# mika314/melonix

Measured on AMD Instinct MI355X. Metric: STFT+pitch+resynth frames/sec (48 kHz, 4096 FFT, 256 hop); % HBM roofline, higher is better.
Workload: dtype f32

## Files before the change

melonix_amd/csrc/stft_core.h:

```cpp
#pragma once
#include <stdint.h>
#include <type_traits>

#if defined(__HIPCC__)
#include <hip/hip_runtime.h>
#define MX_HD __host__ __device__ __forceinline__
namespace mx {
using cpx = float2;
}
#else
#define MX_HD inline __attribute__((always_inline))
namespace mx {
struct alignas(8) cpx {
  float x, y;
};
}
#endif

namespace mx {

#include "stft_consts.inc"

MX_HD cpx mk(float x, float y) {
  cpx r;
// ... 44 lines not shown
  constexpr int k = ((K % 64) + 64) % 64;
  if constexpr (k == 0) {
    pk_bfly_1(E, O, out0, out1);
  } else if constexpr (k == 16) {
    pk_bfly_mi(E, O, out0, out1);
  } else if constexpr (k == 32) {
    pk_bfly_1(E, O, out1, out0);
  } else if constexpr (k == 48) {
    pk_bfly_mi(E, O, out1, out0);
  } else {
    pk_bfly_cs(E, O, mk(kCos64[k], kSin64[k]), out0, out1);
  }
}

template <int R, int Q>
struct Combine {
  static MX_HD void run(const cpx *E, const cpx *O, cpx *out) {
    bfly_w64<Q * 64 / R>(E[Q], O[Q], out[Q], out[Q + R / 2]);
    if constexpr (Q + 1 < R / 2) Combine<R, Q + 1>::run(E, O, out);
  }
};

template <int R>
struct Dft {
  static MX_HD void run(const cpx *in, cpx *out) {
    cpx e[R / 2], o[R / 2], E[R / 2], O[R / 2];
#pragma unroll
    for (int q = 0; q < R / 2; ++q) {
      e[q] = in[2 * q];
      o[q] = in[2 * q + 1];
    }
    Dft<R / 2>::run(e, E);
    Dft<R / 2>::run(o, O);
    Combine<R, 0>::run(E, O, out);
  }
};
template <>
struct Dft<2> {
  static MX_HD void run(const cpx *in, cpx *out) {
    pk_bfly_1(in[0], in[1], out[0], out[1]);
  }
};
template <>
struct Dft<1> {
  static MX_HD void run(const cpx *in, cpx *out) { out[0] = in[0]; }
};

template <int R, int S, int O0, bool CONJ>
struct DftTw {
  static MX_HD void run(const cpx *v, const cpx *w, cpx *out) {
    if constexpr (R == 2) {
      constexpr int i0 = O0, i1 = O0 + S;
      if constexpr (i0 == 0) pk_leaf0_tw<CONJ>(v[0], v[i1], w[i1], out[0], out[1]);
      else pk_leaf_tw<CONJ>(v[i0], w[i0], v[i1], w[i1], out[0], out[1]);
    } else {
      cpx E[R / 2], O[R / 2];
      DftTw<R / 2, 2 * S, O0, CONJ>::run(v, w, E);
      DftTw<R / 2, 2 * S, O0 + S, CONJ>::run(v, w, O);
      Combine<R, 0>::run(E, O, out);
    }
  }
};

template <int N_, int E_>
struct Plan {
  static constexpr int N = N_;
  static constexpr int M = N / 2;
  static constexpr int E = E_;
  static constexpr int T = M / E;
  static constexpr int R3 = E / 2;
  static constexpr int R1 = (N == 4096) ? 16 : 32;
  static constexpr int R2 = M / (R1 * R3);
  static constexpr int NS3 = R1 * R2;
  static constexpr int NB1 = E / R1;
  static constexpr int NB2 = E / R2;
  static constexpr int TW2 = (R2 - 1) * R1;
  static constexpr int TW3 = (R3 - 1) * NS3;
  static constexpr int L1 = ilog2(R1);
  static_assert(N == 4096 || N == 16384 || N == 32768, "supported FFT sizes");
  static_assert((N == 4096) ? E == 16 : E == 32, "supported points per thread");
  static_assert(R1 * R2 * R3 == M && R2 <= E && R1 <= E && T % 64 == 0, "radix plan must cover M");
};

template <class P>
MX_HD constexpr bool t1_padded() { return P::R1 == 32; }
template <class P>
MX_HD constexpr int t1_size() { return t1_padded<P>() ? P::M + P::M / 32 : P::M; }
template <class P>
MX_HD int t1_index(int i) {
  if constexpr (t1_padded<P>()) return i + (i >> 5);
  else return i ^ ((i >> P::L1) & 15);
}

struct alignas(4) f2u {
  float x, y;
};
template <bool ALIGNED8>
MX_HD cpx ld_pair(const float *base, int i) {
  const char *a = reinterpret_cast<const char *>(base) + (size_t)(4u * (unsigned)i);
  if constexpr (ALIGNED8) {
    return *reinterpret_cast<const cpx *>(a);
  } else {
    const f2u u = *reinterpret_cast<const f2u *>(a);
    return mk(u.x, u.y);
  }
}

MX_HD float ld_one(const float *base, int i) {
  return *reinterpret_cast<const float *>(reinterpret_cast<const char *>(base) + (size_t)(4u * (unsigned)i));
}

template <class P, int WSTEP, bool ALIGNED8>
MX_HD void load_frame(int t, cpx (&Y)[P::E], const float *x, const float *w) {
#pragma unroll
  for (int e = 0; e < P::E; ++e) {
    const int p = 2 * (t + P::T * e);
    cpx xs, ws;
    if constexpr (ALIGNED8 && WSTEP == 1) {
      xs = ld_pair<true>(x, p);
      ws = ld_pair<true>(w, p);
    } else {
      xs = ld_pair<false>(x, p);
      if constexpr (WSTEP == 1) {
        ws = ld_pair<false>(w, p);
      } else {
        const f2u wu = *reinterpret_cast<const f2u *>(w - p - 1);
        ws = mk(wu.y, wu.x);
      }
    }
    Y[e] = pk_mul(xs, ws);
  }
}

template <int T>
MX_HD constexpr float win_grow(int e) {
  return T == 64 ? kWinGrow64[e] : T == 128 ? kWinGrow128[e] : T == 256 ? kWinGrow256[e] : kWinGrow512[e];
}
template <class P, bool CLAMP = true>
MX_HD cpx geo_weight(cpx a0, int e) {
  constexpr float sc = 0.5f / (float)P::N;
  const float g = e == 0 ? 1.0f : win_grow<P::T>(e);
  const cpx w = e == 0 ? a0 : mk(a0.x * g, a0.y * g);
  if constexpr (!CLAMP) {
    return w;
  } else {
    const unsigned sb = __builtin_bit_cast(unsigned, sc), xb = __builtin_bit_cast(unsigned, w.x), yb = __builtin_bit_cast(unsigned, w.y);
    return mk(__builtin_bit_cast(float, xb < sb ? xb : sb), __builtin_bit_cast(float, yb < sb ? yb : sb));
  }
}
template <class P>
MX_HD int geo_clamped_slots(int hop) { return (hop + 2 * P::T - 1) / (2 * P::T); }
constexpr int kGeoTail = 2;
template <class P, bool ALIGNED8>
MX_HD void load_frame_geo(int t, cpx (&Y)[P::E], const float *x, const float *wb, int hop) {
  static_assert(P::T == 64 || P::T == 128 || P::T == 256 || P::T == 512, "growth table per T");
  static_assert(P::E <= 32, "growth table length");
  const cpx a0 = ld_pair<true>(wb, 2 * t);
  if (geo_clamped_slots<P>(hop) <= kGeoTail) {
#pragma unroll
    for (int e = 0; e < P::E; ++e) {
      const cpx xs = ld_pair<ALIGNED8>(x, 2 * (t + P::T * e));
      Y[e] = pk_mul(xs, e < P::E - kGeoTail ? geo_weight<P, false>(a0, e) : geo_weight<P, true>(a0, e));
    }
  } else {
#pragma unroll
    for (int e = 0; e < P::E; ++e) Y[e] = pk_mul(ld_pair<ALIGNED8>(x, 2 * (t + P::T * e)), geo_weight<P, true>(a0, e));
  }
}

template <class P>
MX_HD void apply_window_geo(int t, cpx (&Y)[P::E], const cpx (&xr)[P::E], const float *wb, int hop) {
  const cpx a0 = ld_pair<true>(wb, 2 * t);
  if (geo_clamped_slots<P>(hop) <= kGeoTail) {
#pragma unroll
    for (int e = 0; e < P::E; ++e)
      Y[e] = pk_mul(xr[e], e < P::E - kGeoTail ? geo_weight<P, false>(a0, e) : geo_weight<P, true>(a0, e));
  } else {
#pragma unroll
    for (int e = 0; e < P::E; ++e) Y[e] = pk_mul(xr[e], geo_weight<P, true>(a0, e));
  }
}

template <class P, bool ALIGNED8>
MX_HD void load_raw(int t, cpx (&xr)[P::E], const float *x) {
#pragma unroll
  for (int e = 0; e < P::E; ++e) {
    xr[e] = ld_pair<ALIGNED8>(x, 2 * (t + P::T * e));
  }
}
template <class P, int WSTEP, bool ALIGNED8>
MX_HD void apply_window(int t, cpx (&Y)[P::E], const cpx (&xr)[P::E], const float *w) {
#pragma unroll
  for (int e = 0; e < P::E; ++e) {
    const int p = 2 * (t + P::T * e);
    cpx ws;
    if constexpr (WSTEP == 1) {
      ws = ld_pair<ALIGNED8>(w, p);
    } else {
      const f2u wu = *reinterpret_cast<const f2u *>(w - p - 1);
      ws = mk(wu.y, wu.x);
    }
    Y[e] = pk_mul(xr[e], ws);
  }
}

template <class P>
MX_HD void pass1(const cpx (&Y)[P::E], cpx (&v)[P::E]) {
#pragma unroll
  for (int b = 0; b < P::NB1; ++b) {
    cpx in[P::R1], out[P::R1];
#pragma unroll
    for (int r = 0; r < P::R1; ++r) in[r] = Y[b + P::NB1 * r];
    Dft<P::R1>::run(in, out);
#pragma unroll
    for (int r = 0; r < P::R1; ++r) v[b * P::R1 + r] = out[r];
  }
}

template <class P, int HOP>
struct Slide {
  static constexpr int H = HOP / 2;
  static constexpr bool ok = (HOP > 0) && (HOP % 2 == 0) && (H % P::T == 0) && (2 * (H / P::T) <= P::E);
  static constexpr int D = ok ? H / P::T : 1;
};

template <class P, int HOP>
MX_HD void slide_edge(int t, const float *wtab, float inv_sc, cpx (&edge)[Slide<P, HOP>::D]) {
  using S = Slide<P, HOP>;
#pragma unroll
  for (int i = 0; i < S::D; ++i) {
    const int p = 2 * (t + P::T * (P::E - 2 * S::D + i));
    edge[i] = mk(wtab[p] * inv_sc, wtab[p + 1] * inv_sc);
  }
}

template <class P, int HOP>
MX_HD void slide_fetch(int t, const float *xe, cpx (&nx)[Slide<P, HOP>::D]) {
  using S = Slide<P, HOP>;
#pragma unroll
  for (int i = 0; i < S::D; ++i) nx[i] = *reinterpret_cast<const cpx *>(xe - HOP + 2 * (t + P::T * i));
}

template <class P, int HOP>
MX_HD void slide_step(cpx (&Y)[P::E], const cpx (&nx)[Slide<P, HOP>::D], const cpx (&edge)[Slide<P, HOP>::D],
                      float g, float sc) {
  using S = Slide<P, HOP>;
  const cpx gg = mk(g, g), ss = mk(sc, sc);
#pragma unroll
  for (int e = 0; e < P::E - 2 * S::D; ++e) Y[e] = pk_mul_xs(Y[e + S::D], gg);
#pragma unroll
  for (int i = 0; i < S::D; ++i) Y[P::E - 2 * S::D + i] = pk_mul(Y[P::E - S::D + i], edge[i]);
#pragma unroll
  for (int i = 0; i < S::D; ++i) Y[P::E - S::D + i] = pk_mul_xs(nx[i], ss);
}


template <class P>
struct Circ {
  static constexpr int W = 2 * P::T;
  static constexpr int CS = (P::T == 128) ? 4 : (P::T == 256) ? 3 : 2;
  static MX_HD bool ok(int hop) { return hop >= 1 && hop <= (CS - 1) * P::T && hop <= 2 * W; }
  static constexpr int slot(int k) { return (P::E - (CS - 1) + k) & (P::E - 1); }
};
template <class P>
struct CircGeo {
  int o;
  int s;
  int cr;
  int len;
};
template <class P>
MX_HD CircGeo<P> circ_geo(long long frame_end, int hop) {
  constexpr int W = Circ<P>::W;
  const long long start = frame_end - P::N;
  CircGeo<P> g;
  g.o = (int)(start & (long long)(W - 1));
  g.s = ((int)((start - hop) & (long long)(W - 1)) + hop) / W;
  g.len = 2 * hop;
  g.cr = (g.o - g.len) & (P::N - 1);
  return g;
}
template <class P>
MX_HD void circ_load_first(int t, cpx (&Y)[P::E], const float *xa, const float *w, int o) {
#pragma unroll
  for (int e = 0; e < P::E; ++e) {
    const int c2 = 2 * (t + P::T * e);
    const int q0 = (c2 - o) & (P::N - 1), q1 = (c2 + 1 - o) & (P::N - 1);
    Y[e] = mk(xa[q0] * w[q0], xa[q1] * w[q1]);
  }
}
template <class P>
MX_HD void circ_fetch(int t, const float *xs, const float *wt, const CircGeo<P> &g, float (&px)[2 * Circ<P>::CS],
                      float (&pw)[2 * Circ<P>::CS]) {
#pragma unroll
  for (int k = 0; k < Circ<P>::CS; ++k) {
    const int c2 = 2 * (t + P::T * Circ<P>::slot(k));
    int d0 = (c2 - g.cr) & (P::N - 1), d1 = (c2 + 1 - g.cr) & (P::N - 1);
    d0 = d0 < g.len ? d0 : g.len - 1;
    d1 = d1 < g.len ? d1 : g.len - 1;
    px[2 * k] = ld_one(xs, d0);
    px[2 * k + 1] = ld_one(xs, d1);
    pw[2 * k] = ld_one(wt, d0);
    pw[2 * k + 1] = ld_one(wt, d1);
  }
}
template <class P, int S>
MX_HD void circ_age(cpx (&Y)[P::E], cpx gg) {
  cpx head[S > 0 ? S : 1];
#pragma unroll
  for (int i = 0; i < S; ++i) head[i] = Y[i];
#pragma unroll
  for (int e = 0; e < P::E - S; ++e) Y[e] = pk_mul_xs(Y[e + S], gg);
#pragma unroll
  for (int i = 0; i < S; ++i) Y[P::E - S + i] = pk_mul_xs(head[i], gg);
}
template <class P>
MX_HD void circ_step(int t, cpx (&Y)[P::E], float decay, const CircGeo<P> &g, const float (&px)[2 * Circ<P>::CS],
                     const float (&pw)[2 * Circ<P>::CS]) {
  const cpx gg = mk(decay, decay);
  constexpr int SMAX = (Circ<P>::W - 1 + (Circ<P>::CS - 1) * P::T) / Circ<P>::W;
  static_assert(SMAX <= 2, "rotations by 0, 1 or 2 slots");
  if (g.s == 0) circ_age<P, 0>(Y, gg);
  else if (SMAX == 1 || g.s == 1) circ_age<P, 1>(Y, gg);
  else circ_age<P, 2>(Y, gg);
#pragma unroll
  for (int k = 0; k < Circ<P>::CS; ++k) {
    const int e = Circ<P>::slot(k);
    const int c2 = 2 * (t + P::T * e);
    const int d0 = (c2 - g.cr) & (P::N - 1), d1 = (c2 + 1 - g.cr) & (P::N - 1);
    const float n0 = px[2 * k] * pw[2 * k], n1 = px[2 * k + 1] * pw[2 * k + 1];
    Y[e] = mk(d0 < g.len ? n0 : Y[e].x, d1 < g.len ? n1 : Y[e].y);
  }
}


#if defined(__HIP_DEVICE_COMPILE__)
#define MX_LDS_ASM 1
typedef float mx_f2v __attribute__((ext_vector_type(2)));
template <int OFF>
__device__ __forceinline__ mx_f2v lds_rd64(uint32_t addr) {
  static_assert(OFF >= 0 && OFF < 163840, "LDS is 160 KiB");
  mx_f2v r;
  if constexpr (OFF < 65536) {
    asm volatile("ds_read_b64 %0, %1 offset:%2" : "=v"(r) : "v"(addr), "n"(OFF) : "memory");
  } else {
    const uint32_t hi = addr + (uint32_t)(OFF & ~65535);
    asm volatile("ds_read_b64 %0, %1 offset:%2" : "=v"(r) : "v"(hi), "n"(OFF & 65535) : "memory");
  }
  return r;
}
__device__ __forceinline__ uint32_t lds_addr(const void *p) {
  return (uint32_t)(uintptr_t)(const __attribute__((address_space(3))) void *)p;
}
template <int N>
__device__ __forceinline__ void lds_wait(mx_f2v (&q)[N]) {
  static_assert(N % 8 == 0, "tied in groups of 8");
  asm volatile("s_waitcnt lgkmcnt(0)" ::: "memory");
#pragma unroll
  for (int i = 0; i < N; i += 8)
    asm volatile("" : "+v"(q[i]), "+v"(q[i + 1]), "+v"(q[i + 2]), "+v"(q[i + 3]), "+v"(q[i + 4]),
                 "+v"(q[i + 5]), "+v"(q[i + 6]), "+v"(q[i + 7]));
}
#endif
template <int I, int N, class F>
MX_HD void static_for(F &&f) {
  if constexpr (I < N) {
    f(std::integral_constant<int, I>{});
    static_for<I + 1, N>(f);
  }
}

template <class P>
MX_HD void store_t1(int t, const cpx (&v)[P::E], cpx *lds) {
  if constexpr (t1_padded<P>()) {
    static_assert(P::R1 <= 32 && (P::T * P::R1) % 32 == 0, "T1 padding is one point per 32");
    cpx *const p = lds + (t * P::R1 + ((t * P::R1) >> 5));
#pragma unroll
    for (int b = 0; b < P::NB1; ++b) {
#pragma unroll
      for (int r = 0; r < P::R1; ++r) p[b * (P::T * P::R1 + P::T * P::R1 / 32) + r] = v[b * P::R1 + r];
    }
  } else {
    const unsigned B8 = (unsigned)((t * P::R1) ^ (t & 15)) << 3;
    char *const base = reinterpret_cast<char *>(lds);
#pragma unroll
    for (int r = 0; r < P::R1; ++r) {
      cpx *p = reinterpret_cast<cpx *>(base + (B8 ^ ((unsigned)r << 3)));
#pragma unroll
      for (int b = 0; b < P::NB1; ++b) p[b * P::T * P::R1] = v[b * P::R1 + r];
    }
  }
}

template <class P>
struct T1Read {
  static constexpr int S = P::M / P::R2;
  static constexpr int SP = t1_padded<P>() ? S + S / 32 : S;
  static constexpr int TP = t1_padded<P>() ? P::T + P::T / 32 : P::T;
  static constexpr int step = t1_padded<P>() ? 0 : ((S >> P::L1) & 15);
  static_assert(S % 32 == 0 && P::T % 32 == 0 && (step == 0 || step == 8), "T1 read is base(+alt base) + offset");
  static_assert(t1_padded<P>() || P::NB2 == 1, "the XOR layout's bases are written for one pass-2 butterfly per thread");
};

template <class P>
MX_HD void load_t1(int t, cpx (&v)[P::E], const cpx *lds) {
  using R = T1Read<P>;
  const int s1 = t1_index<P>(t);
#ifdef MX_LDS_ASM
  mx_f2v q[P::E];
  const uint32_t ae = lds_addr(lds + s1), ao = lds_addr(lds + (s1 ^ R::step));
  static_for<0, P::NB2>([&](auto bb) {
    constexpr int b = decltype(bb)::value;
    static_for<0, P::R2>([&](auto rr) {
      constexpr int r = decltype(rr)::value;
      q[b * P::R2 + r] = lds_rd64<(b * R::TP + r * R::SP) * 8>((r & 1) ? ao : ae);
    });
  });
  lds_wait(q);
#pragma unroll
  for (int i = 0; i < P::E; ++i) v[i] = mk(q[i].x, q[i].y);
#else
  const cpx *pe = lds + s1, *po = lds + (s1 ^ R::step);
#pragma unroll
  for (int b = 0; b < P::NB2; ++b) {
#pragma unroll
    for (int r = 0; r < P::R2; ++r) v[b * P::R2 + r] = ((r & 1) ? po : pe)[b * R::TP + r * R::SP];
  }
#endif
}

template <class P>
MX_HD void load_t1_tw2(int t, cpx (&v)[P::E], const cpx *lds, const cpx *ltw2, cpx (&w)[P::R2 - 1]) {
  static_assert(P::NB2 == 1 && P::E == P::R2 && P::E % 8 == 0, "one pass-2 butterfly per thread");
  using R = T1Read<P>;
  const int s1 = t1_index<P>(t);
#ifdef MX_LDS_ASM
  const uint32_t ae = lds_addr(lds + s1), ao = lds_addr(lds + (s1 ^ R::step));
  const uint32_t aw = lds_addr(ltw2 + (t & (P::R1 - 1)));
  mx_f2v q[2 * P::E];
  static_for<0, P::R2>([&](auto rr) {
    constexpr int r = decltype(rr)::value;
    q[r] = lds_rd64<r * R::SP * 8>((r & 1) ? ao : ae);
  });
  static_for<1, P::R2>([&](auto rr) {
    constexpr int r = decltype(rr)::value;
    q[P::E + r] = lds_rd64<(r - 1) * P::R1 * 8>(aw);
  });
  q[P::E] = mx_f2v{0.0f, 0.0f};
  lds_wait(q);
#pragma unroll
  for (int i = 0; i < P::E; ++i) v[i] = mk(q[i].x, q[i].y);
#pragma unroll
  for (int r = 1; r < P::R2; ++r) w[r - 1] = mk(q[P::E + r].x, q[P::E + r].y);
#else
  const cpx *pe = lds + s1, *po = lds + (s1 ^ R::step), *pw = ltw2 + (t & (P::R1 - 1));
#pragma unroll
  for (int r = 0; r < P::R2; ++r) v[r] = ((r & 1) ? po : pe)[r * R::SP];
#pragma unroll
  for (int r = 1; r < P::R2; ++r) w[r - 1] = pw[(r - 1) * P::R1];
#endif
}

template <class P>
MX_HD void pass2(int t, cpx (&v)[P::E], const cpx *tw2) {
#pragma unroll
  for (int b = 0; b < P::NB2; ++b) {
    const int j = t + P::T * b;
    const int k = j & (P::R1 - 1);
    cpx in[P::R2], w[P::R2], out[P::R2];
    w[0] = mk(1.0f, 0.0f);
#pragma unroll
    for (int r = 0; r < P::R2; ++r) in[r] = v[b * P::R2 + r];
#pragma unroll
    for (int r = 1; r < P::R2; ++r) {
      w[r] = tw2[(r - 1) * P::R1 + k];
    }
    DftTw<P::R2, 1, 0, false>::run(in, w, out);
#pragma unroll
    for (int r = 0; r < P::R2; ++r) v[b * P::R2 + r] = out[r];
  }
}

template <class P>
MX_HD void pass2_reg(cpx (&v)[P::E], const cpx (&w)[P::R2 - 1]) {
  static_assert(P::NB2 == 1, "one pass-2 butterfly per thread");
  cpx in[P::R2], ww[P::R2], out[P::R2];
  ww[0] = mk(1.0f, 0.0f);
#pragma unroll
  for (int r = 0; r < P::R2; ++r) in[r] = v[r];
#pragma unroll
  for (int r = 1; r < P::R2; ++r) ww[r] = w[r - 1];
  DftTw<P::R2, 1, 0, false>::run(in, ww, out);
#pragma unroll
  for (int r = 0; r < P::R2; ++r) v[r] = out[r];
}

template <class P>
MX_HD void store_t2(int t, const cpx (&v)[P::E], cpx *lds) {
#pragma unroll
  for (int b = 0; b < P::NB2; ++b) {
    const int j = t + P::T * b;
    const int k = j & (P::R1 - 1);
    const int base = (j - k) * P::R2 + k;
    cpx *p = lds + base;
#pragma unroll
    for (int r = 0; r < P::R2; ++r) p[r * P::R1] = v[b * P::R2 + r];
  }
}

template <class P>
MX_HD int k0p(int t) { return t; }
template <class P>
MX_HD int k0q(int t) { return t ? P::NS3 - t : P::NS3 / 2; }

template <class P>
MX_HD void load_t2(int t, cpx (&v)[P::E], const cpx *lds) {
  const int p = k0p<P>(t), q = k0q<P>(t);
#ifdef MX_LDS_ASM
  {
    const uint32_t pa = lds_addr(lds + p), qa = lds_addr(lds + q);
    mx_f2v w[P::E];
    static_for<0, P::R3>([&](auto rr) {
      constexpr int r = decltype(rr)::value;
      w[r] = lds_rd64<P::NS3 * r * 8>(pa);
      w[P::R3 + r] = lds_rd64<P::NS3 * r * 8>(qa);
    });
    lds_wait(w);
#pragma unroll
    for (int i = 0; i < P::E; ++i) v[i] = mk(w[i].x, w[i].y);
  }
#else
  const cpx *pp = lds + p, *qq = lds + q;
#pragma unroll
  for (int r = 0; r < P::R3; ++r) {
    v[r] = pp[P::NS3 * r];
    v[P::R3 + r] = qq[P::NS3 * r];
// ... 242 lines not shown
```

melonix_amd/csrc/stft_kernel_impl.h:

```cpp
#pragma once
#include <hip/hip_runtime.h>

#include "colormap_core.h"
#include "kernels.h"
#include "stft_core.h"
#include "stft_tables.h"

#define MX_BARRIER() __syncthreads()

namespace mx {

template <bool MAXOP>
__device__ __forceinline__ unsigned wave_reduce_u32(unsigned k) {
  constexpr unsigned ident = MAXOP ? 0u : 0xffffffffu;
#define MX_DPP_STEP(CTRL, ROWS)                                                                      \
  {                                                                                                  \
    const unsigned o = (unsigned)__builtin_amdgcn_update_dpp((int)ident, (int)k, CTRL, ROWS, 0xf, false); \
    k = MAXOP ? (o > k ? o : k) : (o < k ? o : k);                                                   \
  }
  MX_DPP_STEP(0xB1, 0xf)
  MX_DPP_STEP(0x4E, 0xf)
  MX_DPP_STEP(0x141, 0xf)
  MX_DPP_STEP(0x140, 0xf)
  MX_DPP_STEP(0x142, 0xa)
  MX_DPP_STEP(0x143, 0xc)
#undef MX_DPP_STEP
  return (unsigned)__builtin_amdgcn_readlane((int)k, 63);
}
__device__ __forceinline__ unsigned long long wave_max_u64(unsigned long long k) {
  const unsigned hi = (unsigned)(k >> 32), lo = (unsigned)k;
  const unsigned mhi = wave_reduce_u32<true>(hi);
  const unsigned long long tie = __ballot(hi == mhi);
  unsigned mlo;
  if (__builtin_popcountll(tie) == 1) mlo = (unsigned)__builtin_amdgcn_readlane((int)lo, __builtin_ctzll(tie));
  else mlo = wave_reduce_u32<true>(hi == mhi ? lo : 0u);
  return ((unsigned long long)mhi << 32) | mlo;
}

template <int IMM, bool NT = true>
__device__ __forceinline__ void st_row_nt(const float *base, unsigned off, float x) {
  static_assert(IMM >= -4096 && IMM <= 4095, "global_store immediate offset");
#if defined(__HIP_DEVICE_COMPILE__)
  if constexpr (NT) asm volatile("global_store_dword %0, %1, %2 offset:%3 nt" : : "v"(off), "v"(x), "s"(base), "n"(IMM) : "memory");
  else asm volatile("global_store_dword %0, %1, %2 offset:%3" : : "v"(off), "v"(x), "s"(base), "n"(IMM) : "memory");
#endif
}

template <class P, int MODE, int HOP, int WPE, bool DEFER = false, bool PREFETCH = false, bool CMAP = false, bool DIRECT = false,
          bool CIRC = false, bool ROWPICK = false>
__global__ __launch_bounds__(P::T) __attribute__((amdgpu_waves_per_eu(WPE, WPE)))
void stft_kernel(const StftArgs a0) {
  const StftArgs &a = a0;
  using C = P;
  constexpr int N = P::N;
  constexpr int NW = C::T / 64;
  constexpr int kRed = (NW > 1) ? ((NW + 1) / 2) * 2 : 0;
  constexpr bool kTw3Bases = (P::R3 == 16);
  constexpr int kTw2 = ((C::TW2 + 1) / 2) * 2;
  static_assert(P::R3 == 16 || P::R3 == 8, "twiddle placement per plan");
  static_assert(!DIRECT || (NW > 1 && !DEFER && !CMAP), "direct row stores: multi-wave, non-deferred plans");
  static_assert(!ROWPICK || (DEFER && NW > 1 && !CMAP && !DIRECT && C::M / 4 / C::T >= 1 && C::T >= 128),
                "row-side pitch pick: the deferred two-wave plan, rows without texels");
  static_assert(!CIRC || (MODE != kRanges && HOP == 0 && !PREFETCH && !CMAP), "circular window: bulk modes");
  constexpr int IMG = t1_size<C>();
  __shared__ __attribute__((aligned(16))) float2 lds[IMG + kRed + (DEFER ? C::M / 2 : 0) + kTw2];
  float *const lout = reinterpret_cast<float *>(DEFER ? lds + IMG : lds);
  float2 *const ltw2 = lds + IMG + kRed + (DEFER ? C::M / 2 : 0);

  const int t_ = threadIdx.x;
  constexpr bool kSlide = (MODE == kBulkAligned) && (HOP > 0) && Slide<P, (HOP > 0 ? HOP : 2)>::ok;
  constexpr int SD = Slide<P, (HOP > 0 ? HOP : 2)>::D;
  const bool wave0 = __builtin_amdgcn_readfirstlane(t_) < 64;
  cpx u[kTw3Bases ? 1 : P::R3];
  cpx ulo;
  cpx w3r[kTw3Bases ? 1 : P::R3 - 1], w3base[6];
  if constexpr (kTw3Bases) {
    cpx uhi_unused;
    post_bases<P>(t_, a.ubase, ulo, uhi_unused);
    fetch_tw3_bases<P>(t_, a.tw3, w3base);
  } else {
    post_twiddles<P>(t_, a.ubase, *reinterpret_cast<cpx(*)[P::R3]>(&u));
    fetch_tw3<P>(t_, a.tw3, *reinterpret_cast<cpx(*)[P::R3 - 1]>(&w3r));
  }
  constexpr int kTw3Hoist = (!kTw3Bases && ROWPICK) ? ((kSlide && SD > 1) ? 3 : P::R3 - 1) : 0;
  cpx w3p[kTw3Hoist > 0 ? kTw3Hoist : 1];
  if constexpr (!kTw3Bases) pass3_wp0<P, kTw3Hoist>(t_, *reinterpret_cast<cpx(*)[P::R3 - 1]>(&w3r), w3p);
  uint32_t bmask_ = 0;
  uint32_t umask = 0;
  if constexpr (!ROWPICK) {
    bmask_ = band_mask<P>(t_, a.kmin, a.kmax);
#pragma unroll
    for (int o = 0; o < P::E; ++o) umask |= (__ballot((bmask_ >> o) & 1u) != 0ull) ? (1u << o) : 0u;
    umask = __builtin_amdgcn_readfirstlane(umask);
  }
  unsigned long long rin[4] = {0ull, 0ull, 0ull, 0ull};
  if constexpr (ROWPICK) {
    const unsigned rm = row_band_mask(4 * t_, a.kmin, a.kmax);
#pragma unroll
    for (int j = 0; j < 4; ++j) rin[j] = __ballot((rm >> j) & 1u);
  }
  constexpr float kSc = 0.5f / (float)N;
  for (int i = t_; i < C::TW2; i += C::T) ltw2[i] = a.tw2[i];
  MX_BARRIER();

  unsigned lb = blockIdx.x;
  {
    const unsigned nb = gridDim.x, xcd = lb & 7u, q = nb >> 3, r = nb & 7u;
    lb = (xcd < r ? xcd * (q + 1) : r * (q + 1) + (xcd - r) * q) + (lb >> 3);
  }
  const int64_t f0 = (int64_t)lb * a.frames_per_block;
  const int64_t f1 = (f0 + a.frames_per_block < a.count) ? f0 + a.frames_per_block : a.count;

  cpx Y[P::E];
  cpx edge[SD], nx[SD];
  if constexpr (kSlide) {
    const int64_t e0 = (a.first_frame + f0 + 1) * (int64_t)HOP;
    if (f0 < f1) load_frame<P, 1, true>(t_, Y, a.audio + MX_AUDIO_PAD + (e0 - N), a.wtab);
    slide_edge<P, HOP>(t_, a.wtab, 2.0f * (float)N, edge);
  }

  unsigned long long *const red = reinterpret_cast<unsigned long long *>(lds + IMG + (DEFER ? C::M / 2 : 0));
  auto flush_pitch = [&](int64_t fr, int tt) {
    if (!ROWPICK && a.pitch && tt == 0) {
      unsigned long long b = red[0];
#pragma unroll
      for (int i = 1; i < NW; ++i) b = red[i] > b ? red[i] : b;
      mx_pitch p;
      p.bin = 0x7fffffff - (int)(unsigned)(b & 0xffffffffull);
      p.mag = __uint_as_float((unsigned)(b >> 32));
      a.pitch[fr] = p;
    }
  };
  const bool want_rows = a.mags != nullptr || (CMAP && a.rgb != nullptr);
  constexpr bool kRowSaddr = (C::M / 4 / C::T == 4) && (C::T * 16 == 2048);
  auto flush_row = [&](int64_t fr, int tt) {
    if (want_rows) {
      using f32x4 = float __attribute__((ext_vector_type(4)));
      const f32x4 *l4 = reinterpret_cast<const f32x4 *>(lout) + tt;
      f32x4 *row4 = reinterpret_cast<f32x4 *>(a.mags + (size_t)fr * (size_t)(N / 2)) + tt;
      f32x4 q[C::M / 4 / C::T];
#pragma unroll
      for (int i = 0; i < C::M / 4 / C::T; ++i) q[i] = l4[C::T * i];
      if (!CMAP || a.mags) {
        if constexpr (kRowSaddr) {
          uintptr_t mid = reinterpret_cast<uintptr_t>(a.mags + (size_t)fr * (size_t)(N / 2)) + 4096;
#if defined(__HIP_DEVICE_COMPILE__)
          asm volatile("" : "+s"(mid));
          using gchar = __attribute__((address_space(1))) char;
          using gf32x4 = __attribute__((address_space(1))) f32x4;
#else
          using gchar = char;
          using gf32x4 = f32x4;
#endif
          const unsigned off = 16u * (unsigned)tt;
#pragma unroll
          for (int i = 0; i < 4; ++i)
            __builtin_nontemporal_store(q[i], reinterpret_cast<gf32x4 *>(reinterpret_cast<gchar *>(mid) + off + (2048 * i - 4096)));
        } else {
#pragma unroll
          for (int i = 0; i < C::M / 4 / C::T; ++i) {
            __builtin_nontemporal_store(q[i], &row4[C::T * i]);
          }
        }
      }
      if constexpr (ROWPICK) {
        if (wave0) {
          const unsigned long long b = wave_max_u64(row_pick_key(
              4 * tt, q[0].x, q[0].y, q[0].z, q[0].w, __builtin_amdgcn_inverse_ballot_w64(rin[0]),
              __builtin_amdgcn_inverse_ballot_w64(rin[1]), __builtin_amdgcn_inverse_ballot_w64(rin[2]),
              __builtin_amdgcn_inverse_ballot_w64(rin[3])));
          if (tt == 0) {
            mx_pitch p;
            p.bin = 0x7fffffff - (int)(unsigned)(b & 0xffffffffull);
            p.mag = __uint_as_float((unsigned)(b >> 32));
            a.pitch[fr] = p;
          }
        }
      }
      if constexpr (CMAP) {
        if (a.rgb) {
          uint32_t *trow = reinterpret_cast<uint32_t *>(a.rgb + (size_t)fr * (size_t)(N / 2) * 3) + 3 * tt;
#pragma unroll 1
          for (int i = 0; i < C::M / 4 / C::T; ++i) {
            uint32_t w3[3];
            texel4(q[i].x, q[i].y, q[i].z, q[i].w, a.cmap_k, w3);
            uint32_t *o = trow + 3 * C::T * i;
            o[0] = w3[0];
            o[1] = w3[1];
            o[2] = w3[2];
          }
        }
      }
    }
  };

  auto frame_ptrs = [&](int64_t fr, int zo, const float *&x, const float *&w) {
    if constexpr (MODE == kRanges) {
      const int s = a.ranges[2 * fr], e = a.ranges[2 * fr + 1];
      const bool outside = (e <= 0) || ((int64_t)e - N >= a.n);
      x = outside ? a.audio : a.audio + MX_AUDIO_PAD + ((int64_t)e - N);
      int64_t d0 = (int64_t)N - ((int64_t)e - (int64_t)s);
      d0 = d0 < (int64_t)(N - 1 - kWOff) ? (int64_t)(N - 1 - kWOff) : d0;
      d0 = d0 > (int64_t)(kWDmax + kWTail) ? (int64_t)(kWDmax + kWTail) : d0;
      w = a.wext + kWOff + d0;
    } else {
      const int64_t e = (a.first_frame + fr + 1) * (int64_t)a.hop;
      x = a.audio + MX_AUDIO_PAD + (e - N);
      w = a.wtab + zo;
    }
  };
  float cpx_[2 * Circ<P>::CS], cpw_[2 * Circ<P>::CS];
  if constexpr (CIRC) {
    if (f0 < f1) {
      const int64_t pe = (a.first_frame + f0 + 1) * (int64_t)a.hop;
      circ_load_first<P>(t_, Y, a.audio + MX_AUDIO_PAD + (pe - N), a.wtab, circ_geo<P>(pe, a.hop).o);
    }
  }
  cpx xr[(PREFETCH && !kSlide) ? P::E : 1];
  if constexpr (PREFETCH && !kSlide) {
    if (f0 < f1) {
      const float *x0;
      const float *w0;
      frame_ptrs(f0, 0, x0, w0);
      load_raw<P, (MODE == kBulkAligned)>(t_, xr, x0);
    }
  }

  for (int64_t f = f0; f < f1; ++f) {
    int t = t_;
    unsigned bmask = bmask_;
    int zoff = 0;
    asm volatile("" : "+v"(t), "+v"(bmask), "+s"(zoff));
    int out_lo, out_hi;
    out_bases<P>(t, out_lo, out_hi);

    if constexpr (CIRC) {
      if (f > f0) {
        const int64_t pe = (a.first_frame + f + 1) * (int64_t)a.hop;
        const CircGeo<P> geo = circ_geo<P>(pe, a.hop);
        circ_fetch<P>(t, a.audio + MX_AUDIO_PAD + (pe - 2 * (int64_t)a.hop), a.wtab + zoff + (N - 2 * a.hop), geo, cpx_, cpw_);
        circ_step<P>(t, Y, a.decay, geo, cpx_, cpw_);
      }
    } else if constexpr (kSlide) {
      if (f > f0) slide_step<P, HOP>(Y, nx, edge, a.decay, kSc);
      if (f + 1 < f1) slide_fetch<P, HOP>(t, a.audio + MX_AUDIO_PAD + (a.first_frame + f + 2) * (int64_t)HOP, nx);
    } else {
      const float *x;
      const float *w;
      frame_ptrs(f, zoff, x, w);
      if constexpr (PREFETCH) {
        if constexpr (MODE == kRanges) apply_window<P, -1, false>(t, Y, xr, w);
        else apply_window_geo<P>(t, Y, xr, a.wtab + N + zoff, a.hop);
      } else if constexpr (MODE == kRanges) {
        load_frame<P, -1, false>(t, Y, x, w);
      } else {
        load_frame_geo<P, (MODE == kBulkAligned)>(t, Y, x, a.wtab + N + zoff, a.hop);
      }
    }

    cpx v[P::E];
    pass1<P>(Y, v);
    constexpr bool kTw2Batch = (P::NB2 == 1);
    store_t1<P>(t, v, lds);
    MX_BARRIER();
    if constexpr (DEFER || DIRECT) {
      if (f > f0) flush_pitch(f - 1, t);
    }
    if constexpr (kTw2Batch) {
      cpx w2[P::R2 - 1];
      load_t1_tw2<P>(t, v, lds, ltw2, w2);
      if constexpr (DEFER) {
        if (f > f0) flush_row(f - 1, t);
      }
      MX_BARRIER();
      pass2_reg<P>(v, w2);
    } else {
      load_t1<P>(t, v, lds);
      if constexpr (DEFER) {
        if (f > f0) flush_row(f - 1, t);
      }
      MX_BARRIER();
      pass2<P>(t, v, ltw2);
    }
    store_t2<P>(t, v, lds);
    MX_BARRIER();
    load_t2<P>(t, v, lds);
    MX_BARRIER();
    float mg[P::E];
    if (NW == 1 || wave0) {
      if constexpr (kTw3Bases) {
        pass3_bases<P, true>(t, v, w3base);
        post_fly<P, true>(t, v, ulo, csel(t == 0, mk(-1.0f, 0.0f), ulo), mg);
      } else {
        pass3_reg<P, true, kTw3Hoist>(t, v, *reinterpret_cast<cpx(*)[P::R3 - 1]>(&w3r), w3p);
        post<P, true>(t, v, *reinterpret_cast<cpx(*)[P::R3]>(&u), mg);
      }
    } else {
      if constexpr (kTw3Bases) {
        pass3_bases<P, false>(t, v, w3base);
        post_fly<P, false>(t, v, ulo, ulo, mg);
      } else {
        pass3_reg<P, false>(t, v, *reinterpret_cast<cpx(*)[P::R3 - 1]>(&w3r));
        post<P, false>(t, v, *reinterpret_cast<cpx(*)[P::R3]>(&u), mg);
      }
    }

    if constexpr (PREFETCH && !kSlide) {
      if (f + 1 < f1) {
        const float *xn;
        const float *wn;
        frame_ptrs(f + 1, zoff, xn, wn);
        load_raw<P, (MODE == kBulkAligned)>(t, xr, xn);
      }
    }

    unsigned long long best = 0ull;
    if (!ROWPICK && a.pitch) {
      const unsigned klo = 0x7fffffffu - (unsigned)out_lo, khi = 0x7fffffffu - (unsigned)out_hi;
      const unsigned nlo = 0x7fffffffu - (unsigned)(C::M - out_lo), nhi = 0x7fffffffu - (unsigned)(C::M - out_hi);
#pragma unroll
      for (int s = 0; s < C::R3; ++s) {
        constexpr int H = C::R3 / 2;
        if (!((umask >> (2 * s)) & 3u)) continue;
        const unsigned b0 = (s < H ? klo : khi) - (unsigned)(C::NS3 * s);
        unsigned b1 = (s < H ? nlo : nhi) + (unsigned)(C::NS3 * s);
        if (s == H) b1 = (t == 0) ? 0x7fffffffu - (unsigned)(C::M / 2) : b1;
        const unsigned v0 = (unsigned)((int)(bmask << (31 - 2 * s)) >> 31);
        const unsigned v1 = (unsigned)((int)(bmask << (31 - (2 * s + 1))) >> 31);
        const unsigned long long k0 = ((unsigned long long)(__float_as_uint(mg[2 * s]) & v0) << 32) | (b0 & v0);
        const unsigned long long k1 = ((unsigned long long)(__float_as_uint(mg[2 * s + 1]) & v1) << 32) | (b1 & v1);
        best = k0 > best ? k0 : best;
        best = k1 > best ? k1 : best;
      }
      best = wave_max_u64(best);
      if constexpr (NW > 1) {
        if ((t & 63) == 0) red[t >> 6] = best;
      }
    }

    if constexpr (DIRECT) {
      if (want_rows) {
        const float *row = a.mags + (size_t)f * (size_t)(N / 2);
        constexpr int H = C::R3 / 2;
        constexpr int STEP = 4 * C::NS3;
        constexpr int G = 8192 / STEP;
        static_assert((STEP == 4096 || STEP == 2048) && H % G == 0, "slot groups share an offset through the store's immediate");
        const unsigned blo = 4u * (unsigned)out_lo, bhi = 4u * (unsigned)(out_hi + C::NS3 * H);
        const unsigned nlo = 4u * (unsigned)(C::M - out_lo), nhi = 4u * (unsigned)(C::M - out_hi - C::NS3 * H);
        static_for<0, C::R3>([&](auto ss) {
          constexpr int s = decltype(ss)::value;
          constexpr int sl = s < H ? s : s - H;
          constexpr int su = (sl & ~(G - 1)) + G / 2, sd = (sl & ~(G - 1)) + G / 2 - 1;
          const unsigned o0 = (s < H ? blo : bhi) + (unsigned)(su * STEP);
          unsigned o1 = (s < H ? nlo : nhi) - (unsigned)(sd * STEP);
          if constexpr (s == H) {
            o1 = (t == 0) ? (unsigned)(4 * (C::M / 2)) + (unsigned)((sl - sd) * STEP) : o1;
          }
          st_row_nt<(sl - su) * STEP>(row, o0, mg[2 * s]);
          st_row_nt<-(sl - sd) * STEP, false>(row, o1, mg[2 * s + 1]);
        });
      }
    } else if (want_rows) {
      float *plo = lout + out_lo, *phi = lout + out_hi;
      float *mlo = lout + (C::M - out_lo), *mhi = lout + (C::M - out_hi);
      constexpr int H = C::R3 / 2;
#pragma unroll
      for (int s = 0; s < C::R3; ++s) (s < H ? plo : phi)[C::NS3 * s] = mg[2 * s];
#pragma unroll
      for (int s = 0; s < C::R3; ++s)
        if (s != H) (s < H ? mlo : mhi)[-C::NS3 * s] = mg[2 * s + 1];
      (t == 0 ? lout + C::M / 2 : mhi - C::NS3 * H)[0] = mg[2 * H + 1];
    }
    if constexpr (!DEFER && !DIRECT) {
      if (want_rows) {
        MX_BARRIER();
        flush_row(f, t);
        MX_BARRIER();
      } else {
        MX_BARRIER();
      }
      if constexpr (NW > 1) {
        flush_pitch(f, t);
      } else if (a.pitch && t == 0) {
        mx_pitch p;
        p.bin = 0x7fffffff - (int)(unsigned)(best & 0xffffffffull);
        p.mag = __uint_as_float((unsigned)(best >> 32));
        a.pitch[f] = p;
      }
    }
  }
  if constexpr (DEFER || DIRECT) {
    if (f0 < f1) {
      MX_BARRIER();
      flush_pitch(f1 - 1, t_);
      if constexpr (DEFER) flush_row(f1 - 1, t_);
    }
  }
}


}
```

Measured before the change: 348.2 million.

## Strength-reduce per-frame addressing and trim LDS twiddle reads in STFT kernel

Replaces the per-frame 64-bit index arithmetic (frame times row size, frame times hop) with pointers that are advanced incrementally, and makes the loop count a wave-uniform int. The row-output test is also turned into a scalar flag. Pass-2 LDS loads now derive the odd-row address by XOR-ing the even address, which relies on an LDS image aligned to 128 bytes, and the padding register is dropped. The geometric window weights are computed once and clamped conditionally, and out_bases is moved to after the passes. Together these aim to cut scalar and vector address math and register pressure in the hot loop, at the cost of more complex pointer bookkeeping.

```diff
diff --git a/melonix_amd/csrc/stft_core.h b/melonix_amd/csrc/stft_core.h
--- a/melonix_amd/csrc/stft_core.h
+++ b/melonix_amd/csrc/stft_core.h
@@ -150,6 +150,22 @@
   static_assert(R1 * R2 * R3 == M && R2 <= E && R1 <= E && T % 64 == 0, "radix plan must cover M");
 };
 
+struct RunState {
+  int n;
+  int64_t f0;
+  int64_t row;
+  int64_t end;
+};
+MX_HD RunState run_setup(int64_t block, int frames_per_block, int64_t count, int64_t first_frame, int hop, int half_row) {
+  RunState r;
+  r.f0 = block * (int64_t)frames_per_block;
+  const int64_t left = count - r.f0;
+  r.n = left <= 0 ? 0 : (left < (int64_t)frames_per_block ? (int)left : frames_per_block);
+  r.row = r.f0 * (int64_t)half_row;
+  r.end = (first_frame + r.f0 + 1) * (int64_t)hop;
+  return r;
+}
+
 template <class P>
 MX_HD constexpr bool t1_padded() { return P::R1 == 32; }
 template <class P>
@@ -204,49 +220,48 @@
 MX_HD constexpr float win_grow(int e) {
   return T == 64 ? kWinGrow64[e] : T == 128 ? kWinGrow128[e] : T == 256 ? kWinGrow256[e] : kWinGrow512[e];
 }
+template <class P>
+MX_HD cpx geo_clamp(cpx w) {
+  constexpr float sc = 0.5f / (float)P::N;
+  const unsigned sb = __builtin_bit_cast(unsigned, sc), xb = __builtin_bit_cast(unsigned, w.x), yb = __builtin_bit_cast(unsigned, w.y);
+  return mk(__builtin_bit_cast(float, xb < sb ? xb : sb), __builtin_bit_cast(float, yb < sb ? yb : sb));
+}
 template <class P, bool CLAMP = true>
 MX_HD cpx geo_weight(cpx a0, int e) {
-  constexpr float sc = 0.5f / (float)P::N;
   const float g = e == 0 ? 1.0f : win_grow<P::T>(e);
   const cpx w = e == 0 ? a0 : mk(a0.x * g, a0.y * g);
-  if constexpr (!CLAMP) {
-    return w;
-  } else {
-    const unsigned sb = __builtin_bit_cast(unsigned, sc), xb = __builtin_bit_cast(unsigned, w.x), yb = __builtin_bit_cast(unsigned, w.y);
-    return mk(__builtin_bit_cast(float, xb < sb ? xb : sb), __builtin_bit_cast(float, yb < sb ? yb : sb));
-  }
+  if constexpr (!CLAMP) return w;
+  else return geo_clamp<P>(w);
 }
 template <class P>
 MX_HD int geo_clamped_slots(int hop) { return (hop + 2 * P::T - 1) / (2 * P::T); }
 constexpr int kGeoTail = 2;
+template <class P>
+MX_HD void geo_window(cpx (&Y)[P::E], const cpx (&xs)[P::E], cpx a0, int hop) {
+  cpx w[P::E];
+#pragma unroll
+  for (int e = 0; e < P::E; ++e) w[e] = e < P::E - kGeoTail ? geo_weight<P, false>(a0, e) : geo_weight<P, true>(a0, e);
+  if (geo_clamped_slots<P>(hop) > kGeoTail) {
+#pragma unroll
+    for (int e = 0; e < P::E - kGeoTail; ++e) w[e] = geo_clamp<P>(w[e]);
+  }
+#pragma unroll
+  for (int e = 0; e < P::E; ++e) Y[e] = pk_mul(xs[e], w[e]);
+}
 template <class P, bool ALIGNED8>
 MX_HD void load_frame_geo(int t, cpx (&Y)[P::E], const float *x, const float *wb, int hop) {
   static_assert(P::T == 64 || P::T == 128 || P::T == 256 || P::T == 512, "growth table per T");
   static_assert(P::E <= 32, "growth table length");
   const cpx a0 = ld_pair<true>(wb, 2 * t);
-  if (geo_clamped_slots<P>(hop) <= kGeoTail) {
-#pragma unroll
-    for (int e = 0; e < P::E; ++e) {
-      const cpx xs = ld_pair<ALIGNED8>(x, 2 * (t + P::T * e));
-      Y[e] = pk_mul(xs, e < P::E - kGeoTail ? geo_weight<P, false>(a0, e) : geo_weight<P, true>(a0, e));
-    }
-  } else {
-#pragma unroll
-    for (int e = 0; e < P::E; ++e) Y[e] = pk_mul(ld_pair<ALIGNED8>(x, 2 * (t + P::T * e)), geo_weight<P, true>(a0, e));
-  }
+  cpx xs[P::E];
+#pragma unroll
+  for (int e = 0; e < P::E; ++e) xs[e] = ld_pair<ALIGNED8>(x, 2 * (t + P::T * e));
+  geo_window<P>(Y, xs, a0, hop);
 }
 
 template <class P>
 MX_HD void apply_window_geo(int t, cpx (&Y)[P::E], const cpx (&xr)[P::E], const float *wb, int hop) {
-  const cpx a0 = ld_pair<true>(wb, 2 * t);
-  if (geo_clamped_slots<P>(hop) <= kGeoTail) {
-#pragma unroll
-    for (int e = 0; e < P::E; ++e)
-      Y[e] = pk_mul(xr[e], e < P::E - kGeoTail ? geo_weight<P, false>(a0, e) : geo_weight<P, true>(a0, e));
-  } else {
-#pragma unroll
-    for (int e = 0; e < P::E; ++e) Y[e] = pk_mul(xr[e], geo_weight<P, true>(a0, e));
-  }
+  geo_window<P>(Y, xr, ld_pair<true>(wb, 2 * t), hop);
 }
 
 template <class P, bool ALIGNED8>
@@ -306,7 +321,7 @@
 MX_HD void slide_fetch(int t, const float *xe, cpx (&nx)[Slide<P, HOP>::D]) {
   using S = Slide<P, HOP>;
 #pragma unroll
-  for (int i = 0; i < S::D; ++i) nx[i] = *reinterpret_cast<const cpx *>(xe - HOP + 2 * (t + P::T * i));
+  for (int i = 0; i < S::D; ++i) nx[i] = ld_pair<true>(xe - HOP, 2 * (t + P::T * i));
 }
 
 template <class P, int HOP>
@@ -422,12 +437,13 @@
 }
 template <int N>
 __device__ __forceinline__ void lds_wait(mx_f2v (&q)[N]) {
-  static_assert(N % 8 == 0, "tied in groups of 8");
   asm volatile("s_waitcnt lgkmcnt(0)" ::: "memory");
 #pragma unroll
-  for (int i = 0; i < N; i += 8)
+  for (int i = 0; i + 8 <= N; i += 8)
     asm volatile("" : "+v"(q[i]), "+v"(q[i + 1]), "+v"(q[i + 2]), "+v"(q[i + 3]), "+v"(q[i + 4]),
                  "+v"(q[i + 5]), "+v"(q[i + 6]), "+v"(q[i + 7]));
+#pragma unroll
+  for (int i = N / 8 * 8; i < N; ++i) asm volatile("" : "+v"(q[i]));
 }
 #endif
 template <int I, int N, class F>
@@ -460,6 +476,7 @@
   }
 }
 
+constexpr int kLdsImageAlign = 128;
 template <class P>
 struct T1Read {
   static constexpr int S = P::M / P::R2;
@@ -497,29 +514,31 @@
 #endif
 }
 
-template <class P>
+template <class P, bool TRIM = false>
 MX_HD void load_t1_tw2(int t, cpx (&v)[P::E], const cpx *lds, const cpx *ltw2, cpx (&w)[P::R2 - 1]) {
   static_assert(P::NB2 == 1 && P::E == P::R2 && P::E % 8 == 0, "one pass-2 butterfly per thread");
   using R = T1Read<P>;
   const int s1 = t1_index<P>(t);
 #ifdef MX_LDS_ASM
-  const uint32_t ae = lds_addr(lds + s1), ao = lds_addr(lds + (s1 ^ R::step));
+  static_assert(kLdsImageAlign % (2 * 8 * (R::step ? R::step : 1)) == 0, "the image's alignment covers the flipped bit");
+  const uint32_t ae = lds_addr(lds + s1), ao = TRIM ? ae ^ (uint32_t)(8 * R::step) : lds_addr(lds + (s1 ^ R::step));
   const uint32_t aw = lds_addr(ltw2 + (t & (P::R1 - 1)));
-  mx_f2v q[2 * P::E];
+  constexpr int PAD = TRIM ? 0 : 1;
+  mx_f2v q[2 * P::E - 1 + PAD];
   static_for<0, P::R2>([&](auto rr) {
     constexpr int r = decltype(rr)::value;
     q[r] = lds_rd64<r * R::SP * 8>((r & 1) ? ao : ae);
   });
   static_for<1, P::R2>([&](auto rr) {
     constexpr int r = decltype(rr)::value;
-    q[P::E + r] = lds_rd64<(r - 1) * P::R1 * 8>(aw);
+    q[P::E + r - 1] = lds_rd64<(r - 1) * P::R1 * 8>(aw);
   });
-  q[P::E] = mx_f2v{0.0f, 0.0f};
+  if constexpr (PAD) q[2 * P::E - 1] = mx_f2v{0.0f, 0.0f};
   lds_wait(q);
 #pragma unroll
   for (int i = 0; i < P::E; ++i) v[i] = mk(q[i].x, q[i].y);
 #pragma unroll
-  for (int r = 1; r < P::R2; ++r) w[r - 1] = mk(q[P::E + r].x, q[P::E + r].y);
+  for (int r = 1; r < P::R2; ++r) w[r - 1] = mk(q[P::E + r - 1].x, q[P::E + r - 1].y);
 #else
   const cpx *pe = lds + s1, *po = lds + (s1 ^ R::step), *pw = ltw2 + (t & (P::R1 - 1));
 #pragma unroll
diff --git a/melonix_amd/csrc/stft_kernel_impl.h b/melonix_amd/csrc/stft_kernel_impl.h
--- a/melonix_amd/csrc/stft_kernel_impl.h
+++ b/melonix_amd/csrc/stft_kernel_impl.h
@@ -63,7 +63,7 @@
                 "row-side pitch pick: the deferred two-wave plan, rows without texels");
   static_assert(!CIRC || (MODE != kRanges && HOP == 0 && !PREFETCH && !CMAP), "circular window: bulk modes");
   constexpr int IMG = t1_size<C>();
-  __shared__ __attribute__((aligned(16))) float2 lds[IMG + kRed + (DEFER ? C::M / 2 : 0) + kTw2];
+  __shared__ __attribute__((aligned(kLdsImageAlign))) float2 lds[IMG + kRed + (DEFER ? C::M / 2 : 0) + kTw2];
   float *const lout = reinterpret_cast<float *>(DEFER ? lds + IMG : lds);
   float2 *const ltw2 = lds + IMG + kRed + (DEFER ? C::M / 2 : 0);
 
@@ -108,19 +108,30 @@
     const unsigned nb = gridDim.x, xcd = lb & 7u, q = nb >> 3, r = nb & 7u;
     lb = (xcd < r ? xcd * (q + 1) : r * (q + 1) + (xcd - r) * q) + (lb >> 3);
   }
-  const int64_t f0 = (int64_t)lb * a.frames_per_block;
-  const int64_t f1 = (f0 + a.frames_per_block < a.count) ? f0 + a.frames_per_block : a.count;
+  const RunState rs = run_setup((int64_t)lb, a.frames_per_block, a.count, a.first_frame, kSlide ? HOP : a.hop, N / 2);
+  const int n = __builtin_amdgcn_readfirstlane(rs.n);
+  constexpr bool kRowSaddr = (C::M / 4 / C::T == 4) && (C::T * 16 == 2048);
+  constexpr int kRowLag = DEFER ? N / 2 : 0, kRowMid = (DEFER && kRowSaddr) ? 1024 : 0;
+  static_assert(!kRowSaddr || DEFER, "the one-base row stores are the deferred plan's");
+  const float *rowp = a.mags + (rs.row - kRowLag + kRowMid);
+  auto *recp = a.pitch + rs.f0;
+  const float *endp = a.audio + MX_AUDIO_PAD + rs.end;
+  int64_t endo = rs.end;
+  const uint64_t rows_p = reinterpret_cast<uintptr_t>(a.mags) | (CMAP ? reinterpret_cast<uintptr_t>(a.rgb) : (uintptr_t)0);
+  unsigned want_rows_ = (unsigned)rows_p | (unsigned)(rows_p >> 32);
+#if defined(__HIP_DEVICE_COMPILE__)
+  asm volatile("" : "+s"(want_rows_));
+#endif
 
   cpx Y[P::E];
   cpx edge[SD], nx[SD];
   if constexpr (kSlide) {
-    const int64_t e0 = (a.first_frame + f0 + 1) * (int64_t)HOP;
-    if (f0 < f1) load_frame<P, 1, true>(t_, Y, a.audio + MX_AUDIO_PAD + (e0 - N), a.wtab);
+    if (n > 0) load_frame<P, 1, true>(t_, Y, endp - N, a.wtab);
     slide_edge<P, HOP>(t_, a.wtab, 2.0f * (float)N, edge);
   }
 
   unsigned long long *const red = reinterpret_cast<unsigned long long *>(lds + IMG + (DEFER ? C::M / 2 : 0));
-  auto flush_pitch = [&](int64_t fr, int tt) {
+  auto flush_pitch = [&](decltype(recp) rec, int tt) {
     if (!ROWPICK && a.pitch && tt == 0) {
       unsigned long long b = red[0];
 #pragma unroll
@@ -128,22 +139,28 @@
       mx_pitch p;
       p.bin = 0x7fffffff - (int)(unsigned)(b & 0xffffffffull);
       p.mag = __uint_as_float((unsigned)(b >> 32));
-      a.pitch[fr] = p;
+      *rec = p;
     }
   };
-  const bool want_rows = a.mags != nullptr || (CMAP && a.rgb != nullptr);
-  constexpr bool kRowSaddr = (C::M / 4 / C::T == 4) && (C::T * 16 == 2048);
-  auto flush_row = [&](int64_t fr, int tt) {
-    if (want_rows) {
+  auto want_rows = [&]() {
+    if constexpr (ROWPICK) return true;
+    unsigned w = want_rows_;
+#if defined(__HIP_DEVICE_COMPILE__)
+    asm volatile("" : "+s"(w));
+#endif
+    return w != 0u;
+  };
+  auto flush_row = [&](const float *row, decltype(recp) rec, int64_t fr, int tt) {
+    if (want_rows()) {
       using f32x4 = float __attribute__((ext_vector_type(4)));
       const f32x4 *l4 = reinterpret_cast<const f32x4 *>(lout) + tt;
-      f32x4 *row4 = reinterpret_cast<f32x4 *>(a.mags + (size_t)fr * (size_t)(N / 2)) + tt;
+      f32x4 *row4 = reinterpret_cast<f32x4 *>(const_cast<float *>(row)) + tt;
       f32x4 q[C::M / 4 / C::T];
 #pragma unroll
       for (int i = 0; i < C::M / 4 / C::T; ++i) q[i] = l4[C::T * i];
       if (!CMAP || a.mags) {
         if constexpr (kRowSaddr) {
-          uintptr_t mid = reinterpret_cast<uintptr_t>(a.mags + (size_t)fr * (size_t)(N / 2)) + 4096;
+          uintptr_t mid = reinterpret_cast<uintptr_t>(row);
 #if defined(__HIP_DEVICE_COMPILE__)
           asm volatile("" : "+s"(mid));
           using gchar = __attribute__((address_space(1))) char;
@@ -173,7 +190,7 @@
             mx_pitch p;
             p.bin = 0x7fffffff - (int)(unsigned)(b & 0xffffffffull);
             p.mag = __uint_as_float((unsigned)(b >> 32));
-            a.pitch[fr] = p;
+            *rec = p;
           }
         }
       }
@@ -194,7 +211,7 @@
     }
   };
 
-  auto frame_ptrs = [&](int64_t fr, int zo, const float *&x, const float *&w) {
+  auto frame_ptrs = [&](int64_t fr, const float *end, int zo, const float *&x, const float *&w) {
     if constexpr (MODE == kRanges) {
       const int s = a.ranges[2 * fr], e = a.ranges[2 * fr + 1];
       const bool outside = (e <= 0) || ((int64_t)e - N >= a.n);
@@ -204,50 +221,45 @@
       d0 = d0 > (int64_t)(kWDmax + kWTail) ? (int64_t)(kWDmax + kWTail) : d0;
       w = a.wext + kWOff + d0;
     } else {
-      const int64_t e = (a.first_frame + fr + 1) * (int64_t)a.hop;
-      x = a.audio + MX_AUDIO_PAD + (e - N);
+      x = end - N;
       w = a.wtab + zo;
     }
   };
   float cpx_[2 * Circ<P>::CS], cpw_[2 * Circ<P>::CS];
   if constexpr (CIRC) {
-    if (f0 < f1) {
-      const int64_t pe = (a.first_frame + f0 + 1) * (int64_t)a.hop;
-      circ_load_first<P>(t_, Y, a.audio + MX_AUDIO_PAD + (pe - N), a.wtab, circ_geo<P>(pe, a.hop).o);
-    }
+    if (n > 0) circ_load_first<P>(t_, Y, endp - N, a.wtab, circ_geo<P>(endo, a.hop).o);
   }
   cpx xr[(PREFETCH && !kSlide) ? P::E : 1];
   if constexpr (PREFETCH && !kSlide) {
-    if (f0 < f1) {
+    if (n > 0) {
       const float *x0;
       const float *w0;
-      frame_ptrs(f0, 0, x0, w0);
+      frame_ptrs(rs.f0, endp, 0, x0, w0);
       load_raw<P, (MODE == kBulkAligned)>(t_, xr, x0);
     }
   }
 
-  for (int64_t f = f0; f < f1; ++f) {
+  for (int i = 0; i < n; ++i) {
+    const int64_t f = rs.f0 + i;
     int t = t_;
     unsigned bmask = bmask_;
     int zoff = 0;
     asm volatile("" : "+v"(t), "+v"(bmask), "+s"(zoff));
     int out_lo, out_hi;
-    out_bases<P>(t, out_lo, out_hi);
 
     if constexpr (CIRC) {
-      if (f > f0) {
-        const int64_t pe = (a.first_frame + f + 1) * (int64_t)a.hop;
-        const CircGeo<P> geo = circ_geo<P>(pe, a.hop);
-        circ_fetch<P>(t, a.audio + MX_AUDIO_PAD + (pe - 2 * (int64_t)a.hop), a.wtab + zoff + (N - 2 * a.hop), geo, cpx_, cpw_);
+      if (i > 0) {
+        const CircGeo<P> geo = circ_geo<P>(endo, a.hop);
+        circ_fetch<P>(t, endp - 2 * a.hop, a.wtab + zoff + (N - 2 * a.hop), geo, cpx_, cpw_);
         circ_step<P>(t, Y, a.decay, geo, cpx_, cpw_);
       }
     } else if constexpr (kSlide) {
-      if (f > f0) slide_step<P, HOP>(Y, nx, edge, a.decay, kSc);
-      if (f + 1 < f1) slide_fetch<P, HOP>(t, a.audio + MX_AUDIO_PAD + (a.first_frame + f + 2) * (int64_t)HOP, nx);
+      if (i > 0) slide_step<P, HOP>(Y, nx, edge, a.decay, kSc);
+      if (i + 1 < n) slide_fetch<P, HOP>(t, endp + HOP, nx);
     } else {
       const float *x;
       const float *w;
-      frame_ptrs(f, zoff, x, w);
+      frame_ptrs(f, endp, zoff, x, w);
       if constexpr (PREFETCH) {
         if constexpr (MODE == kRanges) apply_window<P, -1, false>(t, Y, xr, w);
         else apply_window_geo<P>(t, Y, xr, a.wtab + N + zoff, a.hop);
@@ -264,20 +276,20 @@
     store_t1<P>(t, v, lds);
     MX_BARRIER();
     if constexpr (DEFER || DIRECT) {
-      if (f > f0) flush_pitch(f - 1, t);
+      if (i > 0) flush_pitch(recp - 1, t);
     }
     if constexpr (kTw2Batch) {
       cpx w2[P::R2 - 1];
-      load_t1_tw2<P>(t, v, lds, ltw2, w2);
+      load_t1_tw2<P, true>(t, v, lds, ltw2, w2);
       if constexpr (DEFER) {
-        if (f > f0) flush_row(f - 1, t);
+        if (i > 0) flush_row(rowp, recp - 1, f - 1, t);
       }
       MX_BARRIER();
       pass2_reg<P>(v, w2);
     } else {
       load_t1<P>(t, v, lds);
       if constexpr (DEFER) {
-        if (f > f0) flush_row(f - 1, t);
+        if (i > 0) flush_row(rowp, recp - 1, f - 1, t);
       }
       MX_BARRIER();
       pass2<P>(t, v, ltw2);
@@ -295,7 +307,9 @@
         pass3_reg<P, true, kTw3Hoist>(t, v, *reinterpret_cast<cpx(*)[P::R3 - 1]>(&w3r), w3p);
         post<P, true>(t, v, *reinterpret_cast<cpx(*)[P::R3]>(&u), mg);
       }
+      out_bases<P>(t, out_lo, out_hi);
     } else {
+      out_lo = out_hi = t;
       if constexpr (kTw3Bases) {
         pass3_bases<P, false>(t, v, w3base);
         post_fly<P, false>(t, v, ulo, ulo, mg);
@@ -306,10 +320,10 @@
     }
 
     if constexpr (PREFETCH && !kSlide) {
-      if (f + 1 < f1) {
+      if (i + 1 < n) {
         const float *xn;
         const float *wn;
-        frame_ptrs(f + 1, zoff, xn, wn);
+        frame_ptrs(f + 1, endp + a.hop, zoff, xn, wn);
         load_raw<P, (MODE == kBulkAligned)>(t, xr, xn);
       }
     }
@@ -339,8 +353,8 @@
     }
 
     if constexpr (DIRECT) {
-      if (want_rows) {
-        const float *row = a.mags + (size_t)f * (size_t)(N / 2);
+      if (want_rows()) {
+        const float *row = rowp + kRowLag;
         constexpr int H = C::R3 / 2;
         constexpr int STEP = 4 * C::NS3;
         constexpr int G = 8192 / STEP;
@@ -360,7 +374,7 @@
           st_row_nt<-(sl - sd) * STEP, false>(row, o1, mg[2 * s + 1]);
         });
       }
-    } else if (want_rows) {
+    } else if (want_rows()) {
       float *plo = lout + out_lo, *phi = lout + out_hi;
       float *mlo = lout + (C::M - out_lo), *mhi = lout + (C::M - out_hi);
       constexpr int H = C::R3 / 2;
@@ -372,28 +386,32 @@
       (t == 0 ? lout + C::M / 2 : mhi - C::NS3 * H)[0] = mg[2 * H + 1];
     }
     if constexpr (!DEFER && !DIRECT) {
-      if (want_rows) {
+      if (want_rows()) {
         MX_BARRIER();
-        flush_row(f, t);
+        flush_row(rowp + kRowLag, recp, f, t);
         MX_BARRIER();
       } else {
         MX_BARRIER();
       }
       if constexpr (NW > 1) {
-        flush_pitch(f, t);
+        flush_pitch(recp, t);
       } else if (a.pitch && t == 0) {
         mx_pitch p;
         p.bin = 0x7fffffff - (int)(unsigned)(best & 0xffffffffull);
         p.mag = __uint_as_float((unsigned)(best >> 32));
-        a.pitch[f] = p;
-      }
-    }
+        *recp = p;
+      }
+    }
+    rowp += N / 2;
+    recp += 1;
+    endp += kSlide ? HOP : a.hop;
+    endo += kSlide ? HOP : a.hop;
   }
   if constexpr (DEFER || DIRECT) {
-    if (f0 < f1) {
+    if (n > 0) {
       MX_BARRIER();
-      flush_pitch(f1 - 1, t_);
-      if constexpr (DEFER) flush_row(f1 - 1, t_);
+      flush_pitch(recp - 1, t_);
+      if constexpr (DEFER) flush_row(rowp, recp - 1, rs.f0 + n - 1, t_);
     }
   }
 }
```

Result: no change. 347.2 million (-0.3%).
